# mees/hulc2

Hardware: AMD Instinct MI355X
Metric: play-sequences/sec/node (seq_len=32, 200x200 RGB) (higher is better)
Workload: dtype bf16; 1 GPU; BASELINE configs[1]: synthetic CALVIN-shaped batch, Hulc2.training_step fwd+bwd+allreduce+Adam, static CNN 200x200 + gripper CNN 84x84, lang = random (B,384) embeddings, dropout 0.1, gripper_control on; sequences_per_gpu_step=64, seq_len=32, parallelism=dp1, launch=hipGraph replay (fwd+bwd graph, all-reduce, optimizer graph), frames=fp32 NCHW, already transformed (the reference's dataloader output), gradient_allreduce=none (one rank, no process group), exact_forward_sites=encfc,goal,head,txl

## Files before the change

### hulc2_amd/csrc/gemm.hip

```cpp
#include "hulc_common.h"
#include "hulc_abi_internal.h"
#include <stdlib.h>

namespace {

struct GemmP {
    const void* A; const void* B; void* C;
    const float* bias; const void* add; const void* mask;
    int M, N, K;
    long lda, ldb, ldc, ld_add, ld_mask;
    int a_dtype, b_dtype, c_dtype, add_dtype, mask_dtype;
    int relu, accumulate;
    float alpha, mask_scale, drop_p;
    unsigned long long drop_seed;
    const unsigned long long* seed_dev;
    float* rowsum; int rowsum_accumulate;
};

template <bool KMAJOR, int DT>
HULC_DEVICE void load_operand_chunk_raw(Chunk8& c, const void* base, long ld, int rows, int K, int r, int k0) {
    constexpr int dtype = DT;
    const int kc = k0 < K ? k0 : 0;
    r = r < rows ? r : rows - 1;
    if (KMAJOR) {
        if (dtype == HULC_F32) {
            const float4* q = (const float4*)((const float*)base + (long)r * ld + kc);
            const float4 a = q[0], b = q[1];
            c.v[0] = a.x; c.v[1] = a.y; c.v[2] = a.z; c.v[3] = a.w; c.v[4] = b.x; c.v[5] = b.y; c.v[6] = b.z; c.v[7] = b.w;
        } else {
            const uint4 u = *(const uint4*)((const uint16_t*)base + (long)r * ld + kc);
            c.v[0] = __uint_as_float(u.x); c.v[1] = __uint_as_float(u.y); c.v[2] = __uint_as_float(u.z); c.v[3] = __uint_as_float(u.w);
        }
    } else {
#pragma unroll
        for (int j = 0; j < 8; ++j) {
            const int kk = kc + j < K ? kc + j : 0;
            if (dtype == HULC_F32) c.v[j] = ((const float*)base)[(long)kk * ld + r];
            else c.v[j] = __uint_as_float((unsigned)((const uint16_t*)base)[(long)kk * ld + r]);
        }
    }
}

template <bool KMAJOR, int DT>
HULC_DEVICE void finish_operand_chunk(Chunk8& c, int K, int k0) {
    constexpr int dtype = DT;
    const int nvalid = k0 < K ? K - k0 : 0;
    if (KMAJOR) {
        if (dtype != HULC_F32) {
            const unsigned u[4] = {__float_as_uint(c.v[0]), __float_as_uint(c.v[1]), __float_as_uint(c.v[2]), __float_as_uint(c.v[3])};
#pragma unroll
            for (int j = 0; j < 4; ++j) { c.v[2 * j] = __uint_as_float(u[j] << 16); c.v[2 * j + 1] = __uint_as_float(u[j] & 0xffff0000u); }
        }
        chunk_keep_if(c, nvalid > 0);
    } else {
#pragma unroll
        for (int j = 0; j < 8; ++j) {
            const float v = dtype == HULC_F32 ? c.v[j] : __uint_as_float(__float_as_uint(c.v[j]) << 16);
            c.v[j] = j < nvalid ? v : 0.f;
        }
    }
}

template <int TM, int TN>
HULC_DEVICE void mma_tile_bf16_tr(const char* a_tile, int ra, const char* b_tile, int rb, f32x16_t (&acc)[TM][TN], int lane) {
    typedef short v4s __attribute__((ext_vector_type(4)));
    typedef v4s __attribute__((address_space(3))) * lds_v4s;
    auto tr = [](const char* q) -> v4s { return __builtin_amdgcn_ds_read_tr16_b64_v4i16((lds_v4s)(__attribute__((address_space(3))) char*)q); };
    const int krow = (lane >> 5) * 8 + ((lane & 15) >> 2), col = (((lane >> 4) & 1) * 16 + (lane & 3) * 4) * 2;
#pragma unroll
    for (int ks = 0; ks < 2; ++ks) {
        bf16x8_t a[TM], b[TN];
#pragma unroll
        for (int i = 0; i < TM; ++i) {
            union { v4s v[2]; bf16x8_t f; } x;
            const char* q = a_tile + (ks * 16 + krow) * ra + col + i * 64;
            x.v[0] = tr(q); x.v[1] = tr(q + 4 * ra);
            a[i] = x.f;
        }
#pragma unroll
        for (int j = 0; j < TN; ++j) {
            union { v4s v[2]; bf16x8_t f; } x;
            const char* q = b_tile + (ks * 16 + krow) * rb + col + j * 64;
            x.v[0] = tr(q); x.v[1] = tr(q + 4 * rb);
            b[j] = x.f;
        }
#pragma unroll
        for (int i = 0; i < TM; ++i)
#pragma unroll
            for (int j = 0; j < TN; ++j)
                acc[i][j] = __builtin_amdgcn_mfma_f32_32x32x16_bf16(a[i], b[j], acc[i][j], 0, 0, 0);
    }
}

template <typename CT, int TM, int TN, int WM, int WN, bool AK, bool BK, int ADT, int BDT, bool MICRO>
__global__ __launch_bounds__(WM* WN * 64) void gemm_kernel(GemmP p, float* __restrict__ slabs, int splitk, unsigned* __restrict__ tile_ctr) {
    static_assert(!MICRO || (!AK && !BK), "micro-tile staging is for row-major operands");
    using T = MmaTraits<CT>;
    constexpr int NT = WM * WN * 64;
    constexpr int BM = WM * TM * 32, BN = WN * TN * 32;
// ... 315 lines not shown
                    }
                }
            }
        }
        if (do_rowsum && tid < BM && m0 + tid < p.M) {
            const float* rsl = slabs + (long)splitk * p.M * p.N;
            float v = 0.f;
            for (int z = 0; z < splitk; ++z) v += __hip_atomic_load(rsl + (long)z * p.M + m0 + tid, __ATOMIC_RELAXED, __HIP_MEMORY_SCOPE_AGENT);
            p.rowsum[m0 + tid] = p.rowsum_accumulate ? p.rowsum[m0 + tid] + v : v;
        }
    }

    const unsigned long long seed = p.drop_seed ^ (p.seed_dev ? p.seed_dev[0] : 0ull);
#pragma unroll
    for (int j = 0; j < TN; ++j) {
        const int n = n0 + (wn * TN + j) * 32 + (lane & 31);
        const bool n_ok = n < p.N;
        const int nc = n_ok ? n : 0;
        const float bv = p.bias ? p.bias[nc] : 0.f;
#pragma unroll
        for (int i = 0; i < TM; ++i) {
            float cold[16], addv[16], maskv[16];
#pragma unroll
            for (int e = 0; e < 16; ++e) {
                const int m = m0 + (wm * TM + i) * 32 + acc_row(e, lane);
                const int mc = m < p.M ? m : 0;
                cold[e] = p.accumulate ? load_elem(p.C, p.c_dtype, (long)mc * p.ldc + nc) : 0.f;
                addv[e] = p.add ? load_elem(p.add, p.add_dtype, (long)mc * p.ld_add + nc) : 0.f;
                maskv[e] = p.mask ? load_elem(p.mask, p.mask_dtype, (long)mc * p.ld_mask + nc) : 1.f;
            }
#pragma unroll
            for (int e = 0; e < 16; ++e) {
                const int m = m0 + (wm * TM + i) * 32 + acc_row(e, lane);
                if (m >= p.M || !n_ok) continue;
                float v = p.alpha * acc[i][j][e] + bv + addv[e];
                if (p.relu == 1) v = fmaxf(v, 0.f);
                else if (p.relu == 2) v = 0.5f * v * (1.f + erff(v * 0.70710678118654752f));
                if (p.mask) v = maskv[e] > 0.f ? v * p.mask_scale : 0.f;
                if (p.drop_p > 0.f) v *= dropout_scale(seed, (uint64_t)m * (uint64_t)p.N + n, p.drop_p);
                store_elem(p.C, p.c_dtype, (long)m * p.ldc + n, v + cold[e]);
            }
        }
    }
}


template <typename CT> struct Frag;
template <> struct Frag<bf16_t> {
    bf16x8_t v;
    HULC_DEVICE void set(const Chunk8& c) {
        union { uint4 u; bf16x8_t b; } x;
        x.u.x = pack_bf16x2(c.v[0], c.v[1]); x.u.y = pack_bf16x2(c.v[2], c.v[3]);
        x.u.z = pack_bf16x2(c.v[4], c.v[5]); x.u.w = pack_bf16x2(c.v[6], c.v[7]);
        v = x.b;
    }
};
template <> struct Frag<float> {
    float v[8];
    HULC_DEVICE void set(const Chunk8& c) {
#pragma unroll
        for (int j = 0; j < 8; ++j) v[j] = c.v[j];
    }
};
HULC_DEVICE void frag_mma(const Frag<bf16_t>& a, const Frag<bf16_t>& b, f32x16_t& acc) {
    acc = __builtin_amdgcn_mfma_f32_32x32x16_bf16(a.v, b.v, acc, 0, 0, 0);
}
HULC_DEVICE void frag_mma(const Frag<float>& a, const Frag<float>& b, f32x16_t& acc) {
#pragma unroll
    for (int j = 0; j < 8; ++j) acc = __builtin_amdgcn_mfma_f32_32x32x2f32(a.v[j], b.v[j], acc, 0, 0, 0);
}

HULC_DEVICE float gemm_epilogue(const GemmP& p, float acc, int m, int n) {
    float v = p.alpha * acc + (p.bias ? p.bias[n] : 0.f);
    if (p.add) v += load_elem(p.add, p.add_dtype, (long)m * p.ld_add + n);
    if (p.relu == 1) v = fmaxf(v, 0.f);
    else if (p.relu == 2) v = 0.5f * v * (1.f + erff(v * 0.70710678118654752f));
    if (p.mask) v = load_elem(p.mask, p.mask_dtype, (long)m * p.ld_mask + n) > 0.f ? v * p.mask_scale : 0.f;
    if (p.drop_p > 0.f) v *= dropout_scale(p.drop_seed ^ (p.seed_dev ? p.seed_dev[0] : 0ull), (uint64_t)m * (uint64_t)p.N + n, p.drop_p);
    const long ci = (long)m * p.ldc + n;
    if (p.accumulate) v += load_elem(p.C, p.c_dtype, ci);
    return v;
}

template <typename CT, int TM, bool AK, bool BK, int NW, int ADT, int BDT>
__global__ __launch_bounds__(NW * 64) void gemm_skinny_kernel(GemmP p, float* __restrict__ slabs, int splitk, int kw, unsigned* __restrict__ tile_ctr) {
    __shared__ float red[NW][TM][32][33];
    const int tid = threadIdx.x, lane = tid & 63, wave = tid >> 6;
    const int r = lane & 31, h = lane >> 5;
    const int n0 = blockIdx.x * 32;
    const int kbeg = (blockIdx.y * NW + (wave + blockIdx.x) % NW) * kw;
    int kend = kbeg + kw; if (kend > p.K) kend = p.K;

    f32x16_t acc[TM];
#pragma unroll
    for (int i = 0; i < TM; ++i)
#pragma unroll
        for (int e = 0; e < 16; ++e) acc[i][e] = 0.f;

    constexpr int UN = 4;
    for (int k0 = kbeg; k0 < kend; k0 += 16 * UN) {
        Chunk8 ca[UN][TM], cb[UN];
#pragma unroll
        for (int u = 0; u < UN; ++u) {
            const int k = k0 + u * 16 + h * 8;
#pragma unroll
            for (int i = 0; i < TM; ++i) load_operand_chunk_raw<AK, ADT>(ca[u][i], p.A, p.lda, p.M, kend, i * 32 + r, k);
            load_operand_chunk_raw<BK, BDT>(cb[u], p.B, p.ldb, p.N, kend, n0 + r, k);
        }
#pragma unroll
        for (int u = 0; u < UN; ++u) {
            const int k = k0 + u * 16 + h * 8;
#pragma unroll
            for (int i = 0; i < TM; ++i) finish_operand_chunk<AK, ADT>(ca[u][i], kend, k);
            finish_operand_chunk<BK, BDT>(cb[u], kend, k);
        }
#pragma unroll
        for (int u = 0; u < UN; ++u) {
            Frag<CT> fb; fb.set(cb[u]);
#pragma unroll
            for (int i = 0; i < TM; ++i) { Frag<CT> fa; fa.set(ca[u][i]); frag_mma(fa, fb, acc[i]); }
        }
    }
#pragma unroll
    for (int i = 0; i < TM; ++i)
#pragma unroll
        for (int e = 0; e < 16; ++e) red[wave][i][acc_row(e, lane)][r] = acc[i][e];
    __syncthreads();
    for (int idx = tid; idx < TM * 1024; idx += NW * 64) {
        const int i = idx >> 10, row = (idx >> 5) & 31, col = idx & 31;
        const int m = i * 32 + row, n = n0 + col;
        if (m >= p.M || n >= p.N) continue;
        float v = 0.f;
#pragma unroll
        for (int w = 0; w < NW; ++w) v += red[w][i][row][col];
        if (splitk == 1) store_elem(p.C, p.c_dtype, (long)m * p.ldc + n, gemm_epilogue(p, v, m, n));
        else __hip_atomic_store(slabs + ((long)blockIdx.y * p.M + m) * p.N + n, v, __ATOMIC_RELAXED, __HIP_MEMORY_SCOPE_AGENT);
    }
    if (splitk == 1) return;
    __shared__ int s_last;
    asm volatile("s_waitcnt vmcnt(0)" ::: "memory");
    __syncthreads();
    if (tid == 0) {
        unsigned* c = tile_ctr + blockIdx.x;
        const unsigned old = __hip_atomic_fetch_add(c, 1u, __ATOMIC_RELAXED, __HIP_MEMORY_SCOPE_AGENT);
        const int last = old == (unsigned)(splitk - 1);
        if (last) __hip_atomic_store(c, 0u, __ATOMIC_RELAXED, __HIP_MEMORY_SCOPE_AGENT);
        s_last = last;
    }
    __syncthreads();
    if (!s_last) return;
    for (int idx = tid; idx < TM * 1024; idx += NW * 64) {
        const int i = idx >> 10, row = (idx >> 5) & 31, col = idx & 31;
        const int m = i * 32 + row, n = n0 + col;
        if (m >= p.M || n >= p.N) continue;
        float v = 0.f;
        for (int sl = 0; sl < splitk; ++sl) v += __hip_atomic_load(slabs + ((long)sl * p.M + m) * p.N + n, __ATOMIC_RELAXED, __HIP_MEMORY_SCOPE_AGENT);
        store_elem(p.C, p.c_dtype, (long)m * p.ldc + n, gemm_epilogue(p, v, m, n));
    }
}

constexpr long HULC_GEMM_CTR_BYTES = 16384;

template <typename CT>
void launch_skinny(const GemmP& p, int ak, int bk, float* ws, long ws_bytes, hipStream_t s) {
    const int colblocks = (p.N + 31) / 32;
    const bool big = p.M <= 32 && p.K >= 1024;
    const bool big2 = !big && p.K >= 1024;
    const int nw = big ? 16 : (big2 ? 8 : 4);
    int splitk = 1;
    constexpr int min_kw = 64;
    while (colblocks * splitk < 200 && p.K / (nw * (splitk * 2)) >= min_kw) splitk *= 2;
    unsigned* ctr = (unsigned*)ws;
    ws = ws ? ws + HULC_GEMM_CTR_BYTES / 4 : ws;
    ws_bytes = ws_bytes > HULC_GEMM_CTR_BYTES ? ws_bytes - HULC_GEMM_CTR_BYTES : 0;
    while (splitk > 1 && ((long)splitk * p.M * p.N * 4 > ws_bytes || (long)colblocks * 4 > HULC_GEMM_CTR_BYTES)) splitk /= 2;
    int kw = (p.K + splitk * nw - 1) / (splitk * nw);
    kw = (kw + 15) / 16 * 16;
    dim3 grid(colblocks, splitk);
#define HULC_SK_DT(TMv, AKv, BKv, NWv, ADTv, BDTv) gemm_skinny_kernel<CT, TMv, AKv, BKv, NWv, ADTv, BDTv><<<grid, NWv * 64, 0, s>>>(p, ws, splitk, kw, ctr)
#define HULC_SK(TMv, AKv, BKv, NWv)                                                                         \
    do {                                                                                                    \
        if (sizeof(CT) == 4 || (p.a_dtype == HULC_F32 && p.b_dtype == HULC_F32)) HULC_SK_DT(TMv, AKv, BKv, NWv, HULC_F32, HULC_F32); \
        else if (p.a_dtype == HULC_F32) HULC_SK_DT(TMv, AKv, BKv, NWv, HULC_F32, HULC_BF16);               \
        else if (p.b_dtype == HULC_F32) HULC_SK_DT(TMv, AKv, BKv, NWv, HULC_BF16, HULC_F32);               \
        else HULC_SK_DT(TMv, AKv, BKv, NWv, HULC_BF16, HULC_BF16);                                          \
    } while (0)
    if (big) {
        if (ak && bk) HULC_SK(1, true, true, 16); else if (ak && !bk) HULC_SK(1, true, false, 16);
        else if (!ak && !bk) HULC_SK(1, false, false, 16); else HULC_SK(1, false, true, 16);
    } else if (big2) {
        if (ak && bk) HULC_SK(2, true, true, 8); else if (ak && !bk) HULC_SK(2, true, false, 8);
        else if (!ak && !bk) HULC_SK(2, false, false, 8); else HULC_SK(2, false, true, 8);
    } else if (p.M <= 32) {
        if (ak && bk) HULC_SK(1, true, true, 4); else if (ak && !bk) HULC_SK(1, true, false, 4);
        else if (!ak && !bk) HULC_SK(1, false, false, 4); else HULC_SK(1, false, true, 4);
    } else {
        if (ak && bk) HULC_SK(2, true, true, 4); else if (ak && !bk) HULC_SK(2, true, false, 4);
        else if (!ak && !bk) HULC_SK(2, false, false, 4); else HULC_SK(2, false, true, 4);
    }
#undef HULC_SK_DT
#undef HULC_SK
}

template <typename CT, int TM, int TN, int WM, int WN>
void launch_cfg(const GemmP& p, int ak, int bk, float* ws, long ws_bytes, hipStream_t s) {
    constexpr int BM = WM * TM * 32, BN = WN * TN * 32;
    const int gx = (p.M + BM - 1) / BM, gy = (p.N + BN - 1) / BN;
    const int nkt = (p.K + MmaTraits<CT>::KT - 1) / MmaTraits<CT>::KT;
    int splitk = 1;
    constexpr int target = 768, minkt = 4;
    while (gx * gy * splitk < target && nkt / (splitk * 2) >= minkt) splitk *= 2;
    unsigned* ctr = (unsigned*)ws;
    ws = ws ? ws + HULC_GEMM_CTR_BYTES / 4 : ws;
    ws_bytes = ws_bytes > HULC_GEMM_CTR_BYTES ? ws_bytes - HULC_GEMM_CTR_BYTES : 0;
    while (splitk > 1 && ((long)splitk * p.M * (p.N + 1) * 4 > ws_bytes || (long)gx * gy * 4 > HULC_GEMM_CTR_BYTES)) splitk /= 2;
    dim3 grid(gx, gy, splitk), block(WM * WN * 64);
    const int adt = sizeof(CT) == 4 ? HULC_F32 : p.a_dtype, bdt = sizeof(CT) == 4 ? HULC_F32 : p.b_dtype;
    const int amr = adt == HULC_F32 ? 4 : 8, bmr = bdt == HULC_F32 ? 4 : 8;
    const bool micro = !ak && !bk && p.lda % amr == 0 && p.ldb % bmr == 0 && (uintptr_t)p.A % 16 == 0 && (uintptr_t)p.B % 16 == 0 &&
                       p.M % amr == 0 && p.N % bmr == 0 && p.M >= amr && p.N >= bmr &&
                       (sizeof(CT) == 4 || (p.M % 8 == 0 && p.N % 8 == 0));
#define HULC_GK(AKv, BKv, ADTv, BDTv, MICROv) gemm_kernel<CT, TM, TN, WM, WN, AKv, BKv, ADTv, BDTv, MICROv><<<grid, block, 0, s>>>(p, ws, splitk, ctr)
#define HULC_GK_DT(AKv, BKv, MICROv)                                                              \
    do {                                                                                          \
        if (adt == HULC_F32 && bdt == HULC_F32) HULC_GK(AKv, BKv, HULC_F32, HULC_F32, MICROv);    \
        else if constexpr (sizeof(CT) == 2) {                                                     \
            if (adt == HULC_F32) HULC_GK(AKv, BKv, HULC_F32, HULC_BF16, MICROv);                  \
            else if (bdt == HULC_F32) HULC_GK(AKv, BKv, HULC_BF16, HULC_F32, MICROv);             \
            else HULC_GK(AKv, BKv, HULC_BF16, HULC_BF16, MICROv);                                 \
        }                                                                                         \
    } while (0)
    if (ak && bk) HULC_GK_DT(true, true, false);
    else if (ak && !bk) HULC_GK_DT(true, false, false);
    else if (!ak && bk) HULC_GK_DT(false, true, false);
    else if (micro) HULC_GK_DT(false, false, true);
    else HULC_GK_DT(false, false, false);
#undef HULC_GK_DT
#undef HULC_GK
}

template <typename CT>
void launch_ct(const GemmP& p, int ak, int bk, float* ws, long ws_bytes, hipStream_t s) {
    const long blocks128 = (long)((p.M + 127) / 128) * ((p.N + 127) / 128);
    constexpr int smallk = 256;
    if (blocks128 < 192 || p.K <= smallk) launch_cfg<CT, 1, 1, 2, 2>(p, ak, bk, ws, ws_bytes, s);
    else launch_cfg<CT, 2, 2, 2, 2>(p, ak, bk, ws, ws_bytes, s);
}

}

extern "C" int hulc_gemm(const hulc_gemm_desc* d, void* stream) {
    if (!d || !d->A || !d->B || !d->C) return hulc_fail(-1, "hulc_gemm: null operand");
    if (d->M <= 0 || d->N <= 0 || d->K <= 0) return hulc_fail(-2, "hulc_gemm: non-positive dimension");
    if (d->K % 8 != 0 && (d->a_kmajor || d->b_kmajor)) return hulc_fail(-3, "hulc_gemm: K must be a multiple of 8 for k-major operands");
    const int asz = d->a_dtype == HULC_F32 ? 4 : 2, bsz = d->b_dtype == HULC_F32 ? 4 : 2;
    if (d->a_kmajor && (((uintptr_t)d->A % 16) || (d->lda * asz) % 16)) return hulc_fail(-4, "hulc_gemm: A not 16-byte aligned");
    if (d->b_kmajor && (((uintptr_t)d->B % 16) || (d->ldb * bsz) % 16)) return hulc_fail(-4, "hulc_gemm: B not 16-byte aligned");
    if (d->compute == HULC_F32 && (d->a_dtype != HULC_F32 || d->b_dtype != HULC_F32))
        return hulc_fail(-5, "hulc_gemm: f32 compute requires f32 operands");
    GemmP p;
    p.A = d->A; p.B = d->B; p.C = d->C; p.bias = d->bias; p.add = d->add; p.mask = d->mask;
    p.M = d->M; p.N = d->N; p.K = d->K;
    p.lda = d->lda; p.ldb = d->ldb; p.ldc = d->ldc; p.ld_add = d->ld_add; p.ld_mask = d->ld_mask;
    p.a_dtype = d->a_dtype; p.b_dtype = d->b_dtype; p.c_dtype = d->c_dtype;
    p.add_dtype = d->add_dtype; p.mask_dtype = d->mask_dtype;
    p.relu = d->relu; p.accumulate = d->accumulate;
    p.alpha = d->alpha; p.mask_scale = d->mask_scale; p.drop_p = d->drop_p; p.drop_seed = d->drop_seed;
    p.seed_dev = d->seed_dev;
    p.rowsum = d->rowsum_a; p.rowsum_accumulate = d->rowsum_accumulate;
    if (p.rowsum && d->M <= 64) return hulc_fail(-6, "hulc_gemm: rowsum_a needs M > 64 (tiled path)");
    hipStream_t s = (hipStream_t)stream;
    if (!d->generic_only) {
        const int took = hulc_gemm_tn128_try(d, s);
        if (took < 0) return took;
        if (took) return hulc_check_launch("hulc_gemm");
        const int took2 = hulc_gemm_nt128_try(d, s);
        if (took2 < 0) return took2;
        if (took2) return hulc_check_launch("hulc_gemm");
    }
    if (d->M <= 64) {
        if (d->compute == HULC_F32) launch_skinny<float>(p, d->a_kmajor, d->b_kmajor, (float*)d->ws, d->ws ? d->ws_bytes : 0, s);
        else launch_skinny<bf16_t>(p, d->a_kmajor, d->b_kmajor, (float*)d->ws, d->ws ? d->ws_bytes : 0, s);
    } else if (d->compute == HULC_F32) launch_ct<float>(p, d->a_kmajor, d->b_kmajor, (float*)d->ws, d->ws ? d->ws_bytes : 0, s);
    else launch_ct<bf16_t>(p, d->a_kmajor, d->b_kmajor, (float*)d->ws, d->ws ? d->ws_bytes : 0, s);
    return hulc_check_launch("hulc_gemm");
}
```

### hulc2_amd/kernels.py

```python
import ctypes

import torch

from . import lib as _L
from . import switches

F32, BF16, F16 = (_L.DEFINES["HULC_" + n] for n in ("F32", "BF16", "F16"))
_COMPUTE = {"bf16": BF16, "fp32": F32, "f32": F32}
_compute_mode = BF16


_base_mode = "bf16"
_bwd_mode = None


def set_compute(mode: str) -> None:
    global _compute_mode, _base_mode, _bwd_mode
    if mode not in ("bf16", "fp32", "mixed"):
        raise ValueError(mode)
    _base_mode, _bwd_mode = mode, None
    _compute_mode = _COMPUTE["bf16" if mode == "mixed" else mode]


def get_compute() -> str:
# ... 126 lines not shown
    for t in ts:
        if t is not None and not t.is_cuda:
            raise _L.HulcKernelError(
                "hulc2_amd kernels run on MI355X device memory only; got a CPU tensor "
                "(there is no CPU fallback — use oracle/ for CPU reference values in tests)"
            )


_scratch = {}
_step_state = {}


def step_state(device) -> torch.Tensor:
    t = _step_state.get(device)
    if t is None:
        t = _step_state[device] = torch.tensor([0x243F6A8885A308D3 >> 1, 0], dtype=torch.int64, device=device)
    return t


_rng_fresh = {}
_fault = {}


def fault_word(device) -> torch.Tensor:
    t = _fault.get(device)
    if t is None:
        t = _fault[device] = torch.zeros(1, dtype=torch.int32, device=device)
    return t


def check_faults(device) -> None:
    t = _fault.get(device)
    w = int(t.item()) if t is not None else 0
    if w != 0:
        t.zero_()
        for ws in _chain_ws.values():
            ws.zero_()
        who = [n for b, n in ((1, "rnn_wavefront (HULC_NO_RNN_WAVEFRONT=1 selects the per-step GEMM path)"),
                              (2, "mlp_chain (HULC_NO_MLP_CHAIN=1 selects the per-layer GEMM path)"),
                              (4, "txl_block (HULC_TXL_NO_SHARE=1 keeps one workgroup per sequence, HULC_NO_TXL_BLOCK=1 the per-layer launches)")) if w & b]
        raise _L.HulcKernelError(
            "device-wide barrier timed out in " + " and ".join(who) + " — the kernel's 256 workgroups were not all resident (another "
            "kernel / process shared the GPU, or the device is partitioned).  The optimizer update of that step was skipped.")


_cu_count = {}


def device_cu_count(device) -> int:
    n = _cu_count.get(device)
    if n is None:
        n = _cu_count[device] = torch.cuda.get_device_properties(device).multi_processor_count
    return n


def advance_step_state(device, rng: bool = True, step: bool = True) -> None:
    _call("hulc_step_state_advance_words", step_state(device), rng, step)
    if rng:
        _rng_fresh[device] = True


def ensure_fresh_rng(device) -> None:
    if _rng_fresh.pop(device, False):
        return
    _call("hulc_step_state_advance_words", step_state(device), 1, 0)


def reset_step_state(device, seed: int = 0x243F6A8885A308D3 >> 1, step: int = 0) -> None:
    step_state(device).copy_(torch.tensor([seed, step], dtype=torch.int64))
    _rng_fresh.pop(device, None)



def _gemm_scratch(device) -> torch.Tensor:
    key = (device, torch.cuda.current_stream(device).cuda_stream)
    t = _scratch.get(key)
    if t is None:
        t = _scratch[key] = torch.zeros(8 << 20, dtype=torch.float32, device=device)
    return t


def gemm(A, B, C, M, N, K, lda, ldb, ldc, a_kmajor=True, b_kmajor=True, bias=None, add=None, ld_add=0,
         mask=None, ld_mask=0, mask_scale=1.0, relu=False, accumulate=False, alpha=1.0, drop_p=0.0,
         drop_seed=0, compute=None, rowsum=None, rowsum_accumulate=False, generic_only=False):
    _require_cuda(A, B, C, bias, add, mask)
    d = _L.GemmDesc()
    d.A, d.B, d.C = A.data_ptr(), B.data_ptr(), C.data_ptr()
    d.bias = bias.data_ptr() if bias is not None else None
    d.add = add.data_ptr() if add is not None else None
    d.mask = mask.data_ptr() if mask is not None else None
    d.M, d.N, d.K = M, N, K
    d.lda, d.ldb, d.ldc, d.ld_add, d.ld_mask = lda, ldb, ldc, ld_add, ld_mask
    d.a_dtype, d.b_dtype, d.c_dtype = _dt(A), _dt(B), _dt(C)
    d.add_dtype = _dt(add) if add is not None else F32
    d.mask_dtype = _dt(mask) if mask is not None else F32
    d.a_kmajor, d.b_kmajor = int(a_kmajor), int(b_kmajor)
    d.relu, d.accumulate = int(relu), int(accumulate)
    d.alpha, d.mask_scale, d.drop_p, d.drop_seed = alpha, mask_scale, drop_p, drop_seed
    d.compute = _compute_mode if compute is None else compute
    d.generic_only = int(bool(generic_only))
    if bias is not None and bias.dtype != torch.float32:
        raise TypeError("bias must be float32")
    ws = _gemm_scratch(C.device)
    d.ws, d.ws_bytes = ws.data_ptr(), ws.numel() * 4
    d.seed_dev = step_state(C.device).data_ptr() if drop_p > 0.0 else None
    d.rowsum_a, d.rowsum_accumulate = (rowsum.data_ptr() if rowsum is not None else None), int(rowsum_accumulate)
    esz = lambda t: t.element_size()
    gbytes = M * K * esz(A) + N * K * esz(B) + M * N * esz(C) * (2 if accumulate else 1) \
        + (M * N * esz(add) if add is not None and ld_add else 0) + (M * N * esz(mask) if mask is not None else 0)
    _call("hulc_gemm", ctypes.byref(d), key=("gemm", M, N, K, int(a_kmajor), int(b_kmajor)), flops=2.0 * M * N * K, nbytes=float(gbytes))
    return C


def _conv_desc(N, H, W, Cin, Cout, KH, KW, stride, x_nchw, x_dt, y_dt, w_dt, relu, compute=None):
    d = _L.ConvDesc()
    d.N, d.H, d.W, d.Cin, d.Cout, d.KH, d.KW, d.stride = N, H, W, Cin, Cout, KH, KW, stride
    d.x_nchw, d.x_dtype, d.y_dtype, d.w_dtype, d.relu = int(x_nchw), x_dt, y_dt, w_dt, int(relu)
    d.compute = _compute_mode if compute is None else compute
    return d


def conv_out_hw(H, W, KH, KW, stride):
    return (H - KH) // stride + 1, (W - KW) // stride + 1


def _u8_frames(d, x, aug_shift, aug_pad, frame_index=None):
    if x.dtype != torch.uint8:
        if frame_index is not None:
            raise TypeError("frame_index addresses a uint8 NHWC episode store")
        return
    if frame_index is not None:
        if frame_index.dtype != torch.int32 or not frame_index.is_contiguous() or frame_index.numel() != d.N:
            raise TypeError("frame_index must be a contiguous int32 tensor with one store frame number per batch frame")
        d.frame_index = frame_index.data_ptr()
    if aug_shift is not None and (aug_shift.dtype != torch.int32 or not aug_shift.is_contiguous() or aug_shift.numel() != 2 * d.N):
        raise TypeError("aug_shift must be a contiguous int32 (N, 2) tensor of {sx, sy}")
    d.x_u8_nhwc, d.aug_pad = 1, int(aug_pad)
    d.aug_shift = aug_shift.data_ptr() if aug_shift is not None else None


def _second_frames(d, x, x2, N, Cin, H, W):
    if x2 is None:
        return
    _require_cuda(x2)
    if (x.dtype not in (torch.float32, torch.uint8) or x2.dtype != x.dtype or not x2.is_contiguous() or x2.shape[1:] != x.shape[1:]
            or x.shape[0] + x2.shape[0] != N):
        raise TypeError("x2: a second contiguous frame tensor of x's type and geometry (fp32 NCHW or uint8 NHWC); N = frames of x + frames of x2")
    d.x2, d.n_split = x2.data_ptr(), int(x.shape[0])


_frame_slots = None
_frame_slots_used = set()
_frame_slots_probe = False


def _slot_fields(d, x, x2, H, W, Cin, Cout, KH, stride, x_nchw) -> None:
    if not _frame_slots or not x_nchw or x.dtype != torch.float32 or (Cin, Cout, KH, stride) != (3, 32, 8, 4):
        return
    if W % 4 or (H - 8) % 4 or (W - 8) % 4 or W < 72 or H < 72 or _compute_mode != BF16:
        return
    if _frame_slots_probe:
        if x.data_ptr() in _frame_slots and (x2 is None or x2.data_ptr() in _frame_slots):
            _frame_slots_used.add(x.data_ptr())
            if x2 is not None:
                _frame_slots_used.add(x2.data_ptr())
        return
    a = _frame_slots.get(x.data_ptr())
    b = _frame_slots.get(x2.data_ptr()) if x2 is not None else None
    if a is None or (x2 is not None and b is None):
        return
    d.x_slot = a
    _frame_slots_used.add(x.data_ptr())
    if x2 is not None:
        d.x2_slot = b
        _frame_slots_used.add(x2.data_ptr())


def conv_last_path():
    words = _L.load().hulc_conv_last_path().decode().split()
    if not words:
        return "", {}
    plan = {}
    for w in words[1:]:
# ... 1344 lines not shown
```

### include/hulc2_amd.h

```cpp
#ifndef HULC2_AMD_H
#define HULC2_AMD_H

#ifdef __cplusplus
extern "C" {
#endif

#define HULC_F32 0
#define HULC_BF16 1
#define HULC_F16 2

const char* hulc_last_error(void);
const char* hulc_conv_last_path(void);
int hulc_abi_version(void);
int hulc_stream_create(void** out);

typedef struct {
    const void* A; const void* B; void* C;
    const float* bias; const void* add; const void* mask;
    int M, N, K;
    long lda, ldb, ldc, ld_add, ld_mask;
    int a_dtype, b_dtype, c_dtype, add_dtype, mask_dtype;
    int a_kmajor, b_kmajor;
    int relu, accumulate;
    float alpha, mask_scale, drop_p;
    unsigned long long drop_seed;
    int compute;
    int generic_only;
    void* ws; long ws_bytes;
    const unsigned long long* seed_dev;
    float* rowsum_a; int rowsum_accumulate;
} hulc_gemm_desc;
int hulc_gemm(const hulc_gemm_desc* d, void* stream);


typedef struct {
    int N, H, W, Cin, Cout, KH, KW, stride;
    int x_nchw;
    int x_dtype, y_dtype, w_dtype;
    int relu;
    int compute;
    int dw_oihw;
    int dw_accumulate;
    int x_u8_nhwc;
    int aug_pad;
    const int* aug_shift;
    const int* frame_index;
    void* relu_bits;
    const void* w_lo;
    const void* x2;
    int n_split;
    int conv1_slots;
    const void* x_slot;
    const void* x2_slot;
    void* y_bf16;
} hulc_conv_desc;
int hulc_conv2d_fwd(const hulc_conv_desc* d, const void* x, const void* w, const float* bias, void* y, void* stream);
int hulc_conv2d_bwd_data(const hulc_conv_desc* d, const void* dy, const void* wt, void* dx, const void* relu_src, void* stream);
long hulc_conv2d_bwd_weight_workspace(const hulc_conv_desc* d);
int hulc_conv2d_bwd_weight(const hulc_conv_desc* d, const void* x, const void* dy, float* dw, float* db, void* ws, void* stream);

int hulc_spatial_softmax_fwd(const void* x, int x_dtype, int N, int HW, int C, const float* xmap, const float* ymap,
                             const float* temperature, float* out, float* stats, void* stream);
int hulc_spatial_softmax_bwd(const void* x, int x_dtype, int N, int HW, int C, const float* xmap, const float* ymap,
                             const float* temperature, const float* out, const float* stats, const float* dout,
                             void* dx, int dx_dtype, int relu_mask, void* stream);
int hulc_layernorm_fwd(const float* x, const float* o, float drop_p, unsigned long long seed, const unsigned long long* seed_dev,
                       const float* gamma, const float* beta, float eps, int R, int D, float* pre_out, float* y, float* mean,
                       float* rstd, void* stream);
int hulc_layernorm_slab_fwd(const float* x, const float* o, int n_o, long o_stride, float drop_p, unsigned long long seed,
                            const unsigned long long* seed_dev, const float* gamma, const float* beta, float eps, int R, int D,
                            float* pre_out, float* y, float* mean, float* rstd, void* stream);
int hulc_layernorm_fwd_ld(const float* x, const float* gamma, const float* beta, float eps, int R, int D, float* y, long ld_y, float* mean,
                          float* rstd, void* stream);
int hulc_layernorm_bwd_ld(const float* dy, long ld_dy, const float* pre, const float* mean, const float* rstd, const float* gamma, int R, int D,
                          float* dpre, float* dgamma, float* dbeta, int accumulate_params, void* ws, void* stream);
long hulc_layernorm_bwd_workspace(int R, int D);
int hulc_layernorm_bwd(const float* dy, const float* pre, const float* mean, const float* rstd, const float* gamma, int R, int D,
                       float* dpre, float* do_out, float drop_p, unsigned long long seed, const unsigned long long* seed_dev,
                       float* dgamma, float* dbeta, int accumulate_params, void* ws, void* stream);
long hulc_colsum_workspace(long M, int N);
int hulc_colsum(const void* x, int x_dtype, long M, int N, long ld, float* out, int accumulate, void* ws, void* stream);
int hulc_seq_mean_fwd(const float* x, float* y, int B, int S, int D, float scale, void* stream);
int hulc_seq_mean_bwd(const float* dy, float* dx, int B, int S, int D, void* stream);
int hulc_strided_seq_sum(const void* x, int x_dtype, float* y, int B, int S, int D, long stride_b, long stride_s, long ldy,
                         float scale, void* stream);
int hulc_add_pos_fwd(const float* x, const float* pos, const long* pos_ids, float* y, int B, int S, int D, float drop_p,
                     unsigned long long seed, const unsigned long long* seed_dev, void* stream);
int hulc_dropout_bwd(const float* dy, float* dx, long n, float drop_p, unsigned long long seed, const unsigned long long* seed_dev,
                     void* stream);
int hulc_relu_bwd(const float* dy, const void* y, int y_dtype, float* dx, long n, float scale, void* stream);
int hulc_attention_fwd(const float* qkv, float* out, float* probs, int B, int S, int H, int head_dim, float drop_p,
                       unsigned long long seed, const unsigned long long* seed_dev, void* stream);
int hulc_attention_bwd(const float* qkv, const float* probs, const float* dout, float* dqkv, int B, int S, int H, int head_dim,
                       float drop_p, unsigned long long seed, const unsigned long long* seed_dev, void* stream);

typedef struct {
    int T, A, n_mix, num_classes, nseg;
    long ld;
    float log_scale_min, gripper_alpha;
    const float* act_min; const float* act_max;
    int time_major_B;
} hulc_mix_desc;
long hulc_mix_loss_workspace(const hulc_mix_desc* d);
int hulc_mix_loss_fwd(const hulc_mix_desc* d, const float* y, const float* act, float* out, void* ws, void* stream);
int hulc_mix_loss_bwd(const hulc_mix_desc* d, const float* y, const float* act, const float* gout, float* dy, long ld_dy, void* stream);
int hulc_cat_kl_fwd(const float* pp, const float* pr, int B, int G, int CLS, float beta, int nseg, float* out, float* kl_group, void* stream);
int hulc_cat_kl_bwd(const float* pp, const float* pr, const float* kl_group, int B, int G, int CLS, float beta, float mix,
                    const float* gout, int nseg, float* dpp, float* dpr, void* stream);
int hulc_plan_sample_fwd(const float* logits, const long* idx_in, unsigned long long seed, const unsigned long long* seed_dev,
                         int NG, int CLS, long* idx_out, float* plan, void* stream);
int hulc_plan_sample_bwd(const float* logits, const float* dplan, int NG, int CLS, float* dlogits, int accumulate, void* stream);
int hulc_gauss_plan_fwd(const float* pp, const float* pr, const float* eps_in, unsigned long long seed, const unsigned long long* seed_dev,
                        int B, int P, float min_std, float beta, int nseg, float* plan, float* eps_out, float* out, float* kl_row,
                        void* stream);
int hulc_gauss_plan_bwd(const float* pp, const float* pr, const float* eps_in, unsigned long long seed, const unsigned long long* seed_dev,
// ... 290 lines not shown
```

Before: 20830 play-sequences/s.

## Add one-pass 16x16 skinny GEMM kernel and dispatch rule for mid-M shapes

Adds a new skinny GEMM kernel built on 16x16 MFMA tiles. For M in (32,64] it splits K only across waves inside a workgroup and reduces in LDS, so it needs no split-K slabs or cross-block counters. A rule picks this kernel for small-K or wide-N bf16 shapes, and it runs by default unless the path is overridden. The split-K final reduction is also rewritten to batch slab loads eight at a time, and compile-time-gated timestamp probes are added. The tradeoff is fewer workgroups and less K parallelism on some shapes.

```diff
diff --git a/hulc2_amd/csrc/gemm.hip b/hulc2_amd/csrc/gemm.hip
--- a/hulc2_amd/csrc/gemm.hip
+++ b/hulc2_amd/csrc/gemm.hip
@@ -15,6 +15,9 @@
     unsigned long long drop_seed;
     const unsigned long long* seed_dev;
     float* rowsum; int rowsum_accumulate;
+#ifdef HULC_PROBES
+    unsigned long long* tstamp;
+#endif
 };
 
 template <bool KMAJOR, int DT>
@@ -496,10 +499,26 @@
     return v;
 }
 
-template <typename CT, int TM, bool AK, bool BK, int NW, int ADT, int BDT>
+#ifdef HULC_PROBES
+#define SK_NOW() __builtin_amdgcn_s_memrealtime()
+#define SK_PUT(i_, v_) do { if constexpr (STAMP) { if (tid == 0) p.tstamp[((long)blockIdx.y * gridDim.x + blockIdx.x) * 8 + (i_)] = (v_); } } while (0)
+#define SK_LOADS_ISSUED() do { if constexpr (STAMP) { asm volatile("s_waitcnt vmcnt(0)" ::: "memory"); sk_t1 = SK_NOW(); sk_load += sk_t1 - sk_t0; } } while (0)
+#define SK_BATCH_BEGIN() do { if constexpr (STAMP) sk_t0 = SK_NOW(); } while (0)
+#define SK_BATCH_END(acc_) do { if constexpr (STAMP) { asm volatile("" :: "v"(acc_)); sk_mma += SK_NOW() - sk_t1; } } while (0)
+#else
+#define SK_NOW() 0ull
+#define SK_PUT(i_, v_) do { } while (0)
+#define SK_LOADS_ISSUED() do { } while (0)
+#define SK_BATCH_BEGIN() do { } while (0)
+#define SK_BATCH_END(acc_) do { } while (0)
+#endif
+
+template <typename CT, int TM, bool AK, bool BK, int NW, int ADT, int BDT, bool STAMP = false>
 __global__ __launch_bounds__(NW * 64) void gemm_skinny_kernel(GemmP p, float* __restrict__ slabs, int splitk, int kw, unsigned* __restrict__ tile_ctr) {
     __shared__ float red[NW][TM][32][33];
+    [[maybe_unused]] unsigned long long sk_t0 = 0, sk_t1 = 0, sk_load = 0, sk_mma = 0;
     const int tid = threadIdx.x, lane = tid & 63, wave = tid >> 6;
+    SK_PUT(0, SK_NOW());
     const int r = lane & 31, h = lane >> 5;
     const int n0 = blockIdx.x * 32;
     const int kbeg = (blockIdx.y * NW + (wave + blockIdx.x) % NW) * kw;
@@ -514,6 +533,7 @@
     constexpr int UN = 4;
     for (int k0 = kbeg; k0 < kend; k0 += 16 * UN) {
         Chunk8 ca[UN][TM], cb[UN];
+        SK_BATCH_BEGIN();
 #pragma unroll
         for (int u = 0; u < UN; ++u) {
             const int k = k0 + u * 16 + h * 8;
@@ -521,6 +541,7 @@
             for (int i = 0; i < TM; ++i) load_operand_chunk_raw<AK, ADT>(ca[u][i], p.A, p.lda, p.M, kend, i * 32 + r, k);
             load_operand_chunk_raw<BK, BDT>(cb[u], p.B, p.ldb, p.N, kend, n0 + r, k);
         }
+        SK_LOADS_ISSUED();
 #pragma unroll
         for (int u = 0; u < UN; ++u) {
             const int k = k0 + u * 16 + h * 8;
@@ -534,12 +555,15 @@
 #pragma unroll
             for (int i = 0; i < TM; ++i) { Frag<CT> fa; fa.set(ca[u][i]); frag_mma(fa, fb, acc[i]); }
         }
-    }
+        SK_BATCH_END(acc[TM - 1][0]);
+    }
+    SK_PUT(1, sk_load); SK_PUT(2, sk_mma);
 #pragma unroll
     for (int i = 0; i < TM; ++i)
 #pragma unroll
         for (int e = 0; e < 16; ++e) red[wave][i][acc_row(e, lane)][r] = acc[i][e];
     __syncthreads();
+    SK_PUT(3, SK_NOW());
     for (int idx = tid; idx < TM * 1024; idx += NW * 64) {
         const int i = idx >> 10, row = (idx >> 5) & 31, col = idx & 31;
         const int m = i * 32 + row, n = n0 + col;
@@ -550,10 +574,14 @@
         if (splitk == 1) store_elem(p.C, p.c_dtype, (long)m * p.ldc + n, gemm_epilogue(p, v, m, n));
         else __hip_atomic_store(slabs + ((long)blockIdx.y * p.M + m) * p.N + n, v, __ATOMIC_RELAXED, __HIP_MEMORY_SCOPE_AGENT);
     }
-    if (splitk == 1) return;
+    if (splitk == 1) {
+        if constexpr (STAMP) { asm volatile("s_waitcnt vmcnt(0)" ::: "memory"); SK_PUT(4, SK_NOW()); }
+        return;
+    }
     __shared__ int s_last;
     asm volatile("s_waitcnt vmcnt(0)" ::: "memory");
     __syncthreads();
+    SK_PUT(4, SK_NOW());
     if (tid == 0) {
         unsigned* c = tile_ctr + blockIdx.x;
         const unsigned old = __hip_atomic_fetch_add(c, 1u, __ATOMIC_RELAXED, __HIP_MEMORY_SCOPE_AGENT);
@@ -562,18 +590,167 @@
         s_last = last;
     }
     __syncthreads();
+    SK_PUT(5, SK_NOW()); SK_PUT(7, (unsigned long long)s_last);
     if (!s_last) return;
-    for (int idx = tid; idx < TM * 1024; idx += NW * 64) {
-        const int i = idx >> 10, row = (idx >> 5) & 31, col = idx & 31;
-        const int m = i * 32 + row, n = n0 + col;
+    constexpr int ITER = TM * 1024 / (NW * 64), SW = 8;
+    float vsum[ITER];
+#pragma unroll
+    for (int it = 0; it < ITER; ++it) vsum[it] = 0.f;
+    for (int sl0 = 0; sl0 < splitk; sl0 += SW) {
+        float part[ITER][SW];
+#pragma unroll
+        for (int it = 0; it < ITER; ++it) {
+            const int idx = tid + it * NW * 64;
+            const int m = (idx >> 10) * 32 + ((idx >> 5) & 31), n = n0 + (idx & 31);
+            const int mc = m < p.M ? m : p.M - 1, nc = n < p.N ? n : p.N - 1;
+#pragma unroll
+            for (int j = 0; j < SW; ++j) {
+                const int sl = sl0 + j < splitk ? sl0 + j : splitk - 1;
+                part[it][j] = __hip_atomic_load(slabs + ((long)sl * p.M + mc) * p.N + nc, __ATOMIC_RELAXED, __HIP_MEMORY_SCOPE_AGENT);
+            }
+        }
+#pragma unroll
+        for (int it = 0; it < ITER; ++it)
+#pragma unroll
+            for (int j = 0; j < SW; ++j) vsum[it] += sl0 + j < splitk ? part[it][j] : 0.f;
+    }
+#pragma unroll
+    for (int it = 0; it < ITER; ++it) {
+        const int idx = tid + it * NW * 64;
+        const int m = (idx >> 10) * 32 + ((idx >> 5) & 31), n = n0 + (idx & 31);
+        if (m < p.M && n < p.N) store_elem(p.C, p.c_dtype, (long)m * p.ldc + n, gemm_epilogue(p, vsum[it], m, n));
+    }
+    if constexpr (STAMP) { asm volatile("s_waitcnt vmcnt(0)" ::: "memory"); SK_PUT(6, SK_NOW()); }
+}
+
+HULC_DEVICE void frag_mma16(const Frag<bf16_t>& a, const Frag<bf16_t>& b, f32x4_t& acc) {
+    acc = __builtin_amdgcn_mfma_f32_16x16x32_bf16(a.v, b.v, acc, 0, 0, 0);
+}
+HULC_DEVICE void frag_mma16(const Frag<float>& a, const Frag<float>& b, f32x4_t& acc) {
+#pragma unroll
+    for (int j = 0; j < 8; ++j) acc = __builtin_amdgcn_mfma_f32_16x16x4f32(a.v[j], b.v[j], acc, 0, 0, 0);
+}
+
+constexpr int skinny1p_chunk_dwords(bool kmajor, int dt) { return kmajor && dt != HULC_F32 ? 4 : 8; }
+constexpr int skinny1p_un(bool f32mma, int nw, int tm, bool ak, bool bk, int adt, int bdt) {
+    const int per = tm * skinny1p_chunk_dwords(ak, adt) + skinny1p_chunk_dwords(bk, bdt);
+    const int un = (!(ak && bk) ? 48 : (f32mma ? 96 : 72)) * (16 / nw) / per;
+    return un > 8 ? 8 : (un < 1 ? 1 : un);
+}
+
+template <typename CT, int TM, bool AK, bool BK, int NW, int ADT, int BDT, bool STAMP = false>
+__global__ __launch_bounds__(NW * 64) void gemm_skinny1p_kernel(GemmP p, int kw) {
+    [[maybe_unused]] unsigned long long sk_t0 = 0, sk_t1 = 0, sk_load = 0, sk_mma = 0;
+    constexpr int UN = skinny1p_un(sizeof(CT) == 4, NW, TM, AK, BK, ADT, BDT);
+    __shared__ __attribute__((aligned(16))) float red[NW][TM][256];
+    const int tid = threadIdx.x, lane = tid & 63, wave = tid >> 6;
+    SK_PUT(0, SK_NOW());
+    const int r = lane & 15, g = lane >> 4;
+    const int n0 = blockIdx.x * 16, m0 = blockIdx.y * (TM * 16);
+    const int kbeg = ((wave + blockIdx.x) % NW) * kw;
+    int kend = kbeg + kw; if (kend > p.K) kend = p.K;
+
+    f32x4_t acc[TM];
+#pragma unroll
+    for (int i = 0; i < TM; ++i)
+#pragma unroll
+        for (int e = 0; e < 4; ++e) acc[i][e] = 0.f;
+
+    for (int k0 = kbeg; k0 < kend; k0 += 32 * UN) {
+        Chunk8 ca[UN][TM], cb[UN];
+        SK_BATCH_BEGIN();
+#pragma unroll
+        for (int u = 0; u < UN; ++u) {
+            const int k = k0 + u * 32 + g * 8;
+#pragma unroll
+            for (int i = 0; i < TM; ++i) load_operand_chunk_raw<AK, ADT>(ca[u][i], p.A, p.lda, p.M, kend, m0 + i * 16 + r, k);
+            load_operand_chunk_raw<BK, BDT>(cb[u], p.B, p.ldb, p.N, kend, n0 + r, k);
+        }
+        __builtin_amdgcn_sched_barrier(0);
+        SK_LOADS_ISSUED();
+#pragma unroll
+        for (int u = 0; u < UN; ++u) {
+            const int k = k0 + u * 32 + g * 8;
+#pragma unroll
+            for (int i = 0; i < TM; ++i) finish_operand_chunk<AK, ADT>(ca[u][i], kend, k);
+            finish_operand_chunk<BK, BDT>(cb[u], kend, k);
+        }
+#pragma unroll
+        for (int u = 0; u < UN; ++u) {
+            Frag<CT> fb; fb.set(cb[u]);
+#pragma unroll
+            for (int i = 0; i < TM; ++i) { Frag<CT> fa; fa.set(ca[u][i]); frag_mma16(fa, fb, acc[i]); }
+        }
+        SK_BATCH_END(acc[TM - 1][0]);
+    }
+    SK_PUT(1, sk_load); SK_PUT(2, sk_mma);
+#pragma unroll
+    for (int i = 0; i < TM; ++i) *(f32x4_t*)&red[wave][i][lane * 4] = acc[i];
+    __syncthreads();
+    SK_PUT(3, SK_NOW());
+    for (int idx = tid; idx < TM * 256; idx += NW * 64) {
+        const int i = idx >> 8, row = (idx >> 4) & 15, col = idx & 15;
+        const int m = m0 + i * 16 + row, n = n0 + col;
         if (m >= p.M || n >= p.N) continue;
+        const int at = (row >> 2) * 64 + col * 4 + (row & 3);
         float v = 0.f;
-        for (int sl = 0; sl < splitk; ++sl) v += __hip_atomic_load(slabs + ((long)sl * p.M + m) * p.N + n, __ATOMIC_RELAXED, __HIP_MEMORY_SCOPE_AGENT);
+#pragma unroll
+        for (int w = 0; w < NW; ++w) v += red[w][i][at];
         store_elem(p.C, p.c_dtype, (long)m * p.ldc + n, gemm_epilogue(p, v, m, n));
     }
+    if constexpr (STAMP) { asm volatile("s_waitcnt vmcnt(0)" ::: "memory"); SK_PUT(4, SK_NOW()); }
+}
+
+bool skinny_onepass_rule(int M, int N, int K, int a_dtype, int b_dtype, int compute) {
+    (void)a_dtype; (void)b_dtype;
+    if (M <= 32 || M > 64) return false;
+    if (K <= 128) return N <= 2048;
+    if (compute == HULC_F32 || M <= 48) return false;
+    const int strips = (N + 15) / 16, mtiles = (M + 15) / 16;
+    const int wgs = strips >= 256 ? strips * ((mtiles + 3) / 4) : strips * mtiles;
+    if (wgs > 256) return false;
+    return K <= 2048 && N >= 1024;
 }
 
 constexpr long HULC_GEMM_CTR_BYTES = 16384;
+
+template <typename CT>
+void launch_skinny1p(const GemmP& p, int ak, int bk, hipStream_t s) {
+    const int strips = (p.N + 15) / 16, mtiles = (p.M + 15) / 16;
+    const bool tm4 = strips >= 256 && mtiles > 1;
+    const int nw = tm4 ? 8 : 16;
+    int kw = (p.K + nw - 1) / nw;
+    kw = (kw + 31) / 32 * 32;
+    dim3 grid(strips, tm4 ? (mtiles + 3) / 4 : mtiles);
+#define HULC_S1_DT(TMv, AKv, BKv, ADTv, BDTv) gemm_skinny1p_kernel<CT, TMv, AKv, BKv, (TMv == 4 ? 8 : 16), ADTv, BDTv><<<grid, nw * 64, 0, s>>>(p, kw)
+#define HULC_S1(TMv, AKv, BKv)                                                                              \
+    do {                                                                                                    \
+        if (sizeof(CT) == 4 || (p.a_dtype == HULC_F32 && p.b_dtype == HULC_F32)) HULC_S1_DT(TMv, AKv, BKv, HULC_F32, HULC_F32); \
+        else if constexpr (sizeof(CT) == 2) {                                                               \
+            if (p.a_dtype == HULC_F32) HULC_S1_DT(TMv, AKv, BKv, HULC_F32, HULC_BF16);                     \
+            else if (p.b_dtype == HULC_F32) HULC_S1_DT(TMv, AKv, BKv, HULC_BF16, HULC_F32);                \
+            else HULC_S1_DT(TMv, AKv, BKv, HULC_BF16, HULC_BF16);                                           \
+        }                                                                                                   \
+    } while (0)
+#ifdef HULC_PROBES
+    if (p.tstamp && sizeof(CT) == 2 && ak && bk && p.a_dtype == HULC_F32 && p.b_dtype == HULC_BF16) {
+        if constexpr (sizeof(CT) == 2) {
+            if (tm4) gemm_skinny1p_kernel<CT, 4, true, true, 8, HULC_F32, HULC_BF16, true><<<grid, nw * 64, 0, s>>>(p, kw);
+            else gemm_skinny1p_kernel<CT, 1, true, true, 16, HULC_F32, HULC_BF16, true><<<grid, nw * 64, 0, s>>>(p, kw);
+        }
+        return;
+    }
+#endif
+    if (tm4) {
+        if (ak && bk) HULC_S1(4, true, true); else if (ak && !bk) HULC_S1(4, true, false);
+        else if (!ak && !bk) HULC_S1(4, false, false); else HULC_S1(4, false, true);
+    } else {
+        if (ak && bk) HULC_S1(1, true, true); else if (ak && !bk) HULC_S1(1, true, false);
+        else if (!ak && !bk) HULC_S1(1, false, false); else HULC_S1(1, false, true);
+    }
+#undef HULC_S1_DT
+#undef HULC_S1
+}
 
 template <typename CT>
 void launch_skinny(const GemmP& p, int ak, int bk, float* ws, long ws_bytes, hipStream_t s) {
@@ -599,6 +776,12 @@
         else if (p.b_dtype == HULC_F32) HULC_SK_DT(TMv, AKv, BKv, NWv, HULC_BF16, HULC_F32);               \
         else HULC_SK_DT(TMv, AKv, BKv, NWv, HULC_BF16, HULC_BF16);                                          \
     } while (0)
+#ifdef HULC_PROBES
+    if (p.tstamp && sizeof(CT) == 2 && big2 && ak && bk && p.a_dtype == HULC_F32 && p.b_dtype == HULC_BF16) {
+        if constexpr (sizeof(CT) == 2) gemm_skinny_kernel<CT, 2, true, true, 8, HULC_F32, HULC_BF16, true><<<grid, 8 * 64, 0, s>>>(p, ws, splitk, kw, ctr);
+        return;
+    }
+#endif
     if (big) {
         if (ak && bk) HULC_SK(1, true, true, 16); else if (ak && !bk) HULC_SK(1, true, false, 16);
         else if (!ak && !bk) HULC_SK(1, false, false, 16); else HULC_SK(1, false, true, 16);
@@ -663,6 +846,10 @@
 
 }
 
+extern "C" int hulc_gemm_skinny_onepass(int M, int N, int K, int a_dtype, int b_dtype, int compute) {
+    return skinny_onepass_rule(M, N, K, a_dtype, b_dtype, compute) ? 1 : 0;
+}
+
 extern "C" int hulc_gemm(const hulc_gemm_desc* d, void* stream) {
     if (!d || !d->A || !d->B || !d->C) return hulc_fail(-1, "hulc_gemm: null operand");
     if (d->M <= 0 || d->N <= 0 || d->K <= 0) return hulc_fail(-2, "hulc_gemm: non-positive dimension");
@@ -682,6 +869,10 @@
     p.alpha = d->alpha; p.mask_scale = d->mask_scale; p.drop_p = d->drop_p; p.drop_seed = d->drop_seed;
     p.seed_dev = d->seed_dev;
     p.rowsum = d->rowsum_a; p.rowsum_accumulate = d->rowsum_accumulate;
+#ifdef HULC_PROBES
+    const char* se = getenv("HULC_SK_STAMPS");
+    p.tstamp = se ? (unsigned long long*)strtoull(se, nullptr, 0) : nullptr;
+#endif
     if (p.rowsum && d->M <= 64) return hulc_fail(-6, "hulc_gemm: rowsum_a needs M > 64 (tiled path)");
     hipStream_t s = (hipStream_t)stream;
     if (!d->generic_only) {
@@ -692,7 +883,11 @@
         if (took2 < 0) return took2;
         if (took2) return hulc_check_launch("hulc_gemm");
     }
-    if (d->M <= 64) {
+    if (d->skinny_path < 0 || d->skinny_path > 2) return hulc_fail(-2, "hulc_gemm: skinny_path is 0 (the dispatch rule), 1 (split-K kernel) or 2 (one-pass kernel)");
+    if (d->M <= 64 && (d->skinny_path == 2 || (d->skinny_path == 0 && skinny_onepass_rule(d->M, d->N, d->K, d->a_dtype, d->b_dtype, d->compute)))) {
+        if (d->compute == HULC_F32) launch_skinny1p<float>(p, d->a_kmajor, d->b_kmajor, s);
+        else launch_skinny1p<bf16_t>(p, d->a_kmajor, d->b_kmajor, s);
+    } else if (d->M <= 64) {
         if (d->compute == HULC_F32) launch_skinny<float>(p, d->a_kmajor, d->b_kmajor, (float*)d->ws, d->ws ? d->ws_bytes : 0, s);
         else launch_skinny<bf16_t>(p, d->a_kmajor, d->b_kmajor, (float*)d->ws, d->ws ? d->ws_bytes : 0, s);
     } else if (d->compute == HULC_F32) launch_ct<float>(p, d->a_kmajor, d->b_kmajor, (float*)d->ws, d->ws ? d->ws_bytes : 0, s);
diff --git a/hulc2_amd/kernels.py b/hulc2_amd/kernels.py
--- a/hulc2_amd/kernels.py
+++ b/hulc2_amd/kernels.py
@@ -232,7 +232,7 @@
 
 def gemm(A, B, C, M, N, K, lda, ldb, ldc, a_kmajor=True, b_kmajor=True, bias=None, add=None, ld_add=0,
          mask=None, ld_mask=0, mask_scale=1.0, relu=False, accumulate=False, alpha=1.0, drop_p=0.0,
-         drop_seed=0, compute=None, rowsum=None, rowsum_accumulate=False, generic_only=False):
+         drop_seed=0, compute=None, rowsum=None, rowsum_accumulate=False, generic_only=False, skinny_path=0):
     _require_cuda(A, B, C, bias, add, mask)
     d = _L.GemmDesc()
     d.A, d.B, d.C = A.data_ptr(), B.data_ptr(), C.data_ptr()
@@ -249,6 +249,7 @@
     d.alpha, d.mask_scale, d.drop_p, d.drop_seed = alpha, mask_scale, drop_p, drop_seed
     d.compute = _compute_mode if compute is None else compute
     d.generic_only = int(bool(generic_only))
+    d.skinny_path = int(skinny_path)
     if bias is not None and bias.dtype != torch.float32:
         raise TypeError("bias must be float32")
     ws = _gemm_scratch(C.device)
diff --git a/include/hulc2_amd.h b/include/hulc2_amd.h
--- a/include/hulc2_amd.h
+++ b/include/hulc2_amd.h
@@ -29,8 +29,10 @@
     void* ws; long ws_bytes;
     const unsigned long long* seed_dev;
     float* rowsum_a; int rowsum_accumulate;
+    int skinny_path;
 } hulc_gemm_desc;
 int hulc_gemm(const hulc_gemm_desc* d, void* stream);
+int hulc_gemm_skinny_onepass(int M, int N, int K, int a_dtype, int b_dtype, int compute);
 
 
 typedef struct {
```

Result: faster. 21120 play-sequences/s (median of 6 runs) (+1.4%).
